# alibaba/pairec

Measured on AMD Instinct MI355X. Metric: ranked items/sec, 5k-cand DNN rank (recall top-5000 of 100M x 128 -> DNN3 -> fuse -> sort), higher is better.
Workload: dtype bf16x3; 1 GPU; configs[1]+[2]: recall 5k of 100000000x128 fp32 table in HBM -> 3-layer DNN rank (256-512-256-1, bf16 MFMA with split hi + lo operands = bf16x3, fp32-accurate scores) -> RankScore fusion (fp64) -> ItemRankScore sort; candidates_per_request=5000, table_rows=100000000, dim=128, table_dist=uniform, batches_in_flight=2, contexts=2, all_batches_on_predicted_thresholds=True, batches_re_run_after_a_failed_plan=0, parallelism=1 GPU

## Files before the change

pairec_amd/csrc/common.hpp:

```cpp
#pragma once
#include <hip/hip_runtime.h>

#include <algorithm>
#include <cstdarg>
#include <cstdint>
#include <cstdio>
#include <cstring>
#include <map>
#include <atomic>
#include <memory>
#include <mutex>
#include <shared_mutex>
#include <string>
#include <vector>

#include "../../include/pairec_gpu.h"

namespace pg {

struct PipeRun;
void set_error(const char* fmt, ...);

#define PG_HIP(expr)                                                                           \
    do {                                                                                       \
// ... 423 lines not shown
                      uint32_t* d_out_count);

int rank_dnn3_dev_locked(pg_ctx* ctx, const pg_model* m, const pg_table* t, const float* d_user,
                         const uint32_t* d_cand, const uint32_t* d_off, uint32_t n_req, uint32_t n_items,
                         float* d_out, size_t out_stride = 0);
int fm2t_user_embedding_locked(pg_ctx* ctx, const pg_model* m, const float* d_user, uint32_t n_req, float* d_out);
int rank_fm2t_irows_dev_locked(pg_ctx* ctx, const pg_model* m, const pg_item_rows* ir, const float* d_user, const int32_t* d_ufids,
                               const uint32_t* d_cand, const uint32_t* d_off, uint32_t n_req, uint32_t n_items, float* d_out);
int rank_fm2t_rows_dev_locked(pg_ctx* ctx, const pg_model* m, const pg_features* fs, const int32_t* item_field_cols,
                              const float* d_user, const int32_t* d_ufids, const uint32_t* d_cand, const uint32_t* d_off,
                              uint32_t n_req, uint32_t n_items, float* d_out);
int expr_eval_enqueue_locked(pg_ctx* ctx, const pg_expr* e, const double* d_vars, uint32_t n_items, double* d_out,
                             uint32_t* d_err, uint32_t items_per_flag);
void set_expr_arith_error(const pg_expr* e);
constexpr int kMaxRewrites = 8;
void expr_hold(const pg_expr* e);
void expr_release(const pg_expr* e);
struct ExprHold {
    const pg_expr* e = nullptr;
    ExprHold() = default;
    ExprHold(const ExprHold&) = delete;
    ExprHold& operator=(const ExprHold&) = delete;
    void take(const pg_expr* x) {
        if (e) expr_release(e);
        e = x;
        if (e) expr_hold(e);
    }
    ~ExprHold() { if (e) expr_release(e); }
};
int expr_num_rewrites(const pg_expr* e);
const char* expr_rewrite_source(const pg_expr* e, int r);
int expr_rewrite_num_vars(const pg_expr* e, int r);
const char* expr_rewrite_var_name(const pg_expr* e, int r, int i);
int expr_rewrite_eval_enqueue_locked(pg_ctx* ctx, const pg_expr* e, int r, const double* d_vars, uint32_t n_items, double* d_out,
                                     uint32_t* d_err, uint32_t items_per_flag);
int table_gather_locked(pg_ctx* ctx, const pg_table* t, const uint32_t* d_rows, uint32_t n, float* d_out);
int dpp_run_locked(pg_ctx* ctx, const float* d_emb32, const double* d_hook, const double* d_rel, uint32_t R, uint32_t n,
                   uint32_t d, uint32_t hook_dim, double alpha, uint32_t topn, uint32_t window, int normalize,
                   int ensure_pos, int has_table, uint32_t* d_out, uint32_t* d_out_count, double* d_L_out = nullptr);
int sort_dev_locked(pg_ctx* ctx, const double* d_scores, const uint32_t* d_seg, uint32_t n_seg, uint32_t n_items,
                    uint32_t max_seg, int desc, uint32_t* d_out);

void pipe_pool_destroy(pg_ctx* ctx);
int scratch_reserve(pg_ctx* ctx, int slot, size_t bytes, void** out);
template <class T>
int recall_check(const char* who, const pg_ctx* ctx, const T* over, const void* queries, const void* rows, const void* scores, uint32_t nq,
                 uint32_t k, bool l2) {
    PG_REQUIRE(ctx && over && queries && rows && scores, "%s: NULL argument", who);
    PG_REQUIRE(nq >= 1 && nq <= (uint32_t)kMaxQueries, "%s: nq=%u must be in [1,%d]", who, nq, kMaxQueries);
    PG_REQUIRE(l2 || over->dim <= 128 || nq <= 32, "%s: dim %u supports at most 32 queries per call", who, over->dim);
    if (k < 1 || k > 16384) {
        set_error("%s: k=%u unsupported (1..16384)", who, k);
        return PG_ERR_UNSUPPORTED;
    }
    return PG_OK;
}
template <class Run>
int recall_staged(pg_ctx* ctx, uint32_t dim, const float* queries, uint32_t nq, uint32_t k, uint64_t* out_rows, float* out_scores, Run&& run) {
    void* buf;
    int rc;
    const size_t qb = (size_t)nq * dim * 4, rb = (size_t)nq * k * 8, sb = (size_t)nq * k * 4;
    if ((rc = scratch_reserve(ctx, 5, qb + rb + sb + 64, &buf))) return rc;
    float* d_q = (float*)buf;
    uint64_t* d_rows = (uint64_t*)((char*)buf + ((qb + 15) & ~(size_t)15));
    float* d_sc = (float*)((char*)d_rows + rb);
    PG_HIP(hipMemcpyAsync(d_q, queries, qb, hipMemcpyHostToDevice, ctx->stream));
    if ((rc = run(d_q, d_rows, d_sc))) return rc;
    PG_HIP(hipMemcpyAsync(out_rows, d_rows, rb, hipMemcpyDeviceToHost, ctx->stream));
// ... 9 lines not shown
```

pairec_amd/csrc/expr.hip:

```cpp
#include "common.hpp"

#include <cmath>
#include <string>
#include <vector>

namespace pg {

enum OpCode : uint32_t { OP_CONST = 0, OP_VAR, OP_ADD, OP_SUB, OP_MUL, OP_DIV, OP_MOD, OP_POW, OP_FNZ,
                         OP_DIVF,
                         OP_NEG };

struct Instr {
    uint32_t op;
    uint32_t arg;
    double val;
};

constexpr int kMaxStack = 32;
constexpr int kMaxProg = 128;

}

struct pg_expr {
    std::string source;
// ... 233 lines not shown
    if (xfin && x != 0.0 && x != 1.0 && y != 0.0 && ay < 9223372036854775808.0 && ay == trunc(ay)) {
        double a1 = 1.0;
        long long ae = 0;
        int xe_i;
        double x1 = frexp(x, &xe_i);
        long long xe = xe_i;
        for (long long i = (long long)ay; i != 0; i >>= 1) {
            if (xe < -(1ll << 12) || (1ll << 12) < xe) {
                ae += xe;
                break;
            }
            if (i & 1) {
                a1 *= x1;
                ae += xe;
            }
            x1 *= x1;
            xe <<= 1;
            if (x1 < 0.5) {
                x1 += x1;
                xe--;
            }
        }
        if (y < 0.0) {
            a1 = 1.0 / a1;
            ae = -ae;
        }
        if (ae > 4096) ae = 4096;
        if (ae < -4096) ae = -4096;
        return ldexp(a1, (int)ae);
    }
    return pow(x, y);
}

__global__ void expr_eval_kernel(ExprDev e, const double* __restrict__ vars, uint32_t n_items,
                                 double* __restrict__ out, uint32_t* __restrict__ err, uint32_t items_per_flag) {
    const uint32_t i = blockIdx.x * blockDim.x + threadIdx.x;
    if (i >= n_items) return;
    double st[kMaxStack];
    int sp = 0;
    bool bad = false;
    for (uint32_t pc = 0; pc < e.n; ++pc) {
        const Instr in = e.prog[pc];
        if (in.op == OP_CONST) {
            st[sp++] = in.val;
        } else if (in.op == OP_VAR) {
            st[sp++] = vars[(size_t)in.arg * n_items + i];
        } else {
            if (in.op == OP_NEG) {
                st[sp - 1] = -st[sp - 1];
                continue;
            }
            const double r = st[--sp];
            const double l = st[--sp];
            double v = 0.0;
            switch (in.op) {
                case OP_DIVF: v = l / r; break;
                case OP_ADD: v = l + r; break;
                case OP_SUB: v = l - r; break;
                case OP_MUL: v = l * r; break;
                case OP_DIV:
                    if (r == 0.0) bad = true; else v = l / r;
                    break;
                case OP_MOD: {
                    const long long li = (l == l && fabs(l) < 9223372036854775808.0) ? (long long)l : (long long)0x8000000000000000ull;
                    const long long ri = (r == r && fabs(r) < 9223372036854775808.0) ? (long long)r : (long long)0x8000000000000000ull;
                    if (ri == 0) bad = true;
                    else if (ri == -1) v = 0.0;
                    else v = (double)(li % ri);
                    break;
                }
                case OP_POW: v = go_pow(l, r); break;
                case OP_FNZ: v = (l != 0.0) ? l : r; break;
            }
            st[sp++] = v;
        }
    }
    out[i] = sp > 0 ? st[sp - 1] : 0.0;
    if (bad) atomicOr(err + (items_per_flag ? i / items_per_flag : 0u), 1u);
}

int expr_eval_enqueue_locked(pg_ctx* ctx, const pg_expr* e, const double* d_vars, uint32_t n_items, double* d_out,
                             uint32_t* d_err, uint32_t items_per_flag) {
    if (e->empty) {
        PG_HIP(hipMemsetAsync(d_out, 0, (size_t)n_items * 8, ctx->stream));
    } else {
        ExprDev dev;
        dev.n = (uint32_t)e->prog.size();
        for (size_t i = 0; i < e->prog.size(); ++i) dev.prog[i] = e->prog[i];
        expr_eval_kernel<<<(n_items + 255) / 256, 256, 0, ctx->stream>>>(dev, d_vars, n_items, d_out, d_err, items_per_flag);
        PG_HIP(hipGetLastError());
    }
    return PG_OK;
}

int expr_num_rewrites(const pg_expr* e) { return e ? (int)e->rewrites.size() : 0; }
const char* expr_rewrite_source(const pg_expr* e, int r) { return e->rewrites[(size_t)r].source.c_str(); }
int expr_rewrite_num_vars(const pg_expr* e, int r) { return (int)e->rewrites[(size_t)r].vars.size(); }
const char* expr_rewrite_var_name(const pg_expr* e, int r, int i) { return e->rewrites[(size_t)r].vars[(size_t)i].c_str(); }
int expr_rewrite_eval_enqueue_locked(pg_ctx* ctx, const pg_expr* e, int r, const double* d_vars, uint32_t n_items, double* d_out,
                                     uint32_t* d_err, uint32_t items_per_flag) {
    const pg_expr::Rewrite& rw = e->rewrites[(size_t)r];
    if (rw.failed || rw.prog.empty()) {
        PG_HIP(hipMemsetAsync(d_out, 0, (size_t)n_items * 8, ctx->stream));
        return PG_OK;
    }
    ExprDev dev;
    dev.n = (uint32_t)rw.prog.size();
    for (size_t i = 0; i < rw.prog.size(); ++i) dev.prog[i] = rw.prog[i];
    expr_eval_kernel<<<(n_items + 255) / 256, 256, 0, ctx->stream>>>(dev, d_vars, n_items, d_out, d_err, items_per_flag);
    PG_HIP(hipGetLastError());
    return PG_OK;
}

void set_expr_arith_error(const pg_expr* e) {
    set_error("pg_expr_eval: violation of arithmetic specification: a division by zero in '%s' "
              "(the reference panics in ExprASTResult, utils/ast/ast.go:243-249)", e->source.c_str());
}

static int expr_eval_locked(pg_ctx* ctx, const pg_expr* e, const double* d_vars, uint32_t n_items,
                            double* d_out) {
    void* p;
    int rc;
    if ((rc = scratch_reserve(ctx, 4, 4096, &p))) return rc;
    uint32_t* d_err = (uint32_t*)p + 320;
    PG_HIP(hipMemsetAsync(d_err, 0, 4, ctx->stream));
    if ((rc = expr_eval_enqueue_locked(ctx, e, d_vars, n_items, d_out, d_err, 0))) return rc;
    PG_HIP(hipMemcpyAsync(ctx->h_status + 320, d_err, 4, hipMemcpyDeviceToHost, ctx->stream));
    PG_HIP(hipStreamSynchronize(ctx->stream));
    if (ctx->h_status[320] != 0) {
        set_expr_arith_error(e);
        return PG_ERR_ARITH;
    }
    return PG_OK;
}

struct ExprCol {
    const void* base;
    int32_t dtype;
    int32_t pad;
    double def;
};
struct ExprCols16 { ExprCol c[16]; };
// ... 353 lines not shown
```

pairec_amd/csrc/misc.hip:

```cpp
#include "pipeline.hpp"

#include <algorithm>
#include <cstring>
#include <vector>

namespace pg {

__global__ void rows_to_local_kernel(const uint64_t* __restrict__ rows, uint32_t n, uint64_t off,
                                     uint64_t nrows, uint32_t* __restrict__ local,
                                     uint8_t* __restrict__ owned, uint32_t* __restrict__ uni_off, uint32_t uni_nq, uint32_t uni_k) {
    const uint32_t i = blockIdx.x * blockDim.x + threadIdx.x;
    if (uni_off && i <= uni_nq) uni_off[i] = i * uni_k;
    if (i >= n) return;
    const uint64_t r = rows[i];
    const bool mine = r != ~0ull && r >= off && r - off < nrows;
    local[i] = mine ? (uint32_t)(r - off) : 0u;
    if (owned) owned[i] = mine ? 1 : 0;
}

__global__ void widen_kernel(const float* __restrict__ in, uint32_t n, double* __restrict__ out) {
    const uint32_t i = blockIdx.x * blockDim.x + threadIdx.x;
    if (i < n) out[i] = (double)in[i];
}

typedef uint32_t u32x4 __attribute__((ext_vector_type(4)));
__global__ __launch_bounds__(256) void hbm_probe_kernel(const u32x4* __restrict__ p, uint64_t n16,
                                                        uint32_t* __restrict__ sink) {
    uint32_t acc = 0;
    const uint64_t stride = (uint64_t)gridDim.x * blockDim.x;
    uint64_t i = (uint64_t)blockIdx.x * blockDim.x + threadIdx.x;
    for (; i + 3 * stride < n16; i += 4 * stride) {
        const u32x4 a = __builtin_nontemporal_load(&p[i]);
        const u32x4 b = __builtin_nontemporal_load(&p[i + stride]);
        const u32x4 c = __builtin_nontemporal_load(&p[i + 2 * stride]);
        const u32x4 d = __builtin_nontemporal_load(&p[i + 3 * stride]);
        acc ^= a.x ^ a.y ^ a.z ^ a.w ^ b.x ^ b.y ^ b.z ^ b.w ^ c.x ^ c.y ^ c.z ^ c.w ^ d.x ^ d.y ^ d.z ^ d.w;
    }
    for (; i < n16; i += stride) {
        const u32x4 a = __builtin_nontemporal_load(&p[i]);
        acc ^= a.x ^ a.y ^ a.z ^ a.w;
    }
    if (acc == 0x9E3779B9u) *sink = acc;
}

__global__ void uniform_offsets_kernel(uint32_t nq, uint32_t k, uint32_t* __restrict__ off) {
// ... 53 lines not shown
    sorted_head_kernel<<<(nq * C + 255) / 256, 256, 0, st>>>(d_order, d_rows, d_fused, nq, k, C, d_c_rows, d_c_rel);
    PG_HIP(hipGetLastError());
    return PG_OK;
}

int gather_global_rows_launch(hipStream_t st, const pg_table* t, const uint64_t* d_global_rows, uint32_t n, float* d_out) {
    if (n == 0) return PG_OK;
    const uint64_t threads = (uint64_t)n * (t->dim / 4);
    gather_global_rows_kernel<<<(uint32_t)((threads + 255) / 256), 256, 0, st>>>(t->d, t->dim, t->row_offset, t->rows, d_global_rows, n, d_out);
    PG_HIP(hipGetLastError());
    return PG_OK;
}

size_t page_entry_bytes(int n_algos) { return 20 + 4 * (size_t)n_algos; }

int page_launch(hipStream_t st, const uint32_t* d_order, const uint32_t* d_pick, const uint32_t* d_pick_cnt,
                const uint64_t* d_rows, const float* d_recall, const float* d_rank, size_t rank_stride, int n_algos,
                const double* d_fused, uint32_t nq, uint32_t k, uint32_t top_n, char* d_page) {
    const size_t np = (size_t)nq * top_n;
    if (np == 0) return PG_OK;
    uint64_t* p_rows = (uint64_t*)d_page;
    double* p_fused = (double*)(p_rows + np);
    float* p_recall = (float*)(p_fused + np);
    float* p_rank = p_recall + np;
    page_kernel<<<(uint32_t)((np + 255) / 256), 256, 0, st>>>(d_order, d_pick, d_pick_cnt, d_rows, d_recall, d_rank, rank_stride, n_algos,
                                                             d_fused, nq, k, top_n, p_rows, p_fused, p_recall, p_rank);
    PG_HIP(hipGetLastError());
    return PG_OK;
}

int rows_to_local_locked(pg_ctx* ctx, const pg_table* t, const uint64_t* d_rows, uint32_t n, uint32_t* d_local,
                         uint8_t* d_owned) {
    if (n == 0) return PG_OK;
    rows_to_local_kernel<<<(n + 255) / 256, 256, 0, ctx->stream>>>(d_rows, n, t->row_offset, t->rows, d_local, d_owned, nullptr, 0, 0);
    PG_HIP(hipGetLastError());
    return PG_OK;
}

int rows_to_local_offsets_locked(pg_ctx* ctx, const pg_table* t, const uint64_t* d_rows, uint32_t nq, uint32_t k, uint32_t* d_local,
                                 uint32_t* d_off) {
    const uint32_t n = nq * k;
    if (n <= nq) {
        int rc = uniform_offsets_locked(ctx, nq, k, d_off);
        return rc ? rc : rows_to_local_locked(ctx, t, d_rows, n, d_local, nullptr);
    }
    rows_to_local_kernel<<<(n + 255) / 256, 256, 0, ctx->stream>>>(d_rows, n, t->row_offset, t->rows, d_local, nullptr, d_off, nq, k);
    PG_HIP(hipGetLastError());
    return PG_OK;
}

int uniform_offsets_locked(pg_ctx* ctx, uint32_t nq, uint32_t k, uint32_t* d_off) {
    uniform_offsets_kernel<<<(nq + 256) / 256, 256, 0, ctx->stream>>>(nq, k, d_off);
    PG_HIP(hipGetLastError());
    return PG_OK;
}

}

extern "C" {

int pg_hbm_read_probe(pg_ctx* ctx, const pg_table* t, int reps, double* out_gbps) {
    PG_REQUIRE(ctx && t && out_gbps && reps > 0, "pg_hbm_read_probe: bad argument");
    const void* d_buf = t->d;
    const uint64_t bytes = t->rows * (uint64_t)t->dim * 4;
    PG_REQUIRE(bytes >= (1u << 20), "pg_hbm_read_probe: table smaller than 1 MiB");
    std::lock_guard<std::mutex> g(ctx->mu);
    void* sink;
    int rc;
    if ((rc = pg::scratch_reserve(ctx, 4, 4096, &sink))) return rc;
    const uint64_t n16 = bytes / 16;
    const int grid = ctx->num_cus * 8;
    double best = 0.0;
    for (int r = 0; r < reps + 1; ++r) {
        PG_HIP(hipEventRecord(ctx->ev[0], ctx->stream));
        pg::hbm_probe_kernel<<<grid, 256, 0, ctx->stream>>>((const pg::u32x4*)d_buf, n16, (uint32_t*)sink + 900);
        PG_HIP(hipGetLastError());
        PG_HIP(hipEventRecord(ctx->ev[1], ctx->stream));
        PG_HIP(hipStreamSynchronize(ctx->stream));
        float ms = 0.f;
// ... 27 lines not shown
```

pairec_amd/csrc/pipeline.hip:

```cpp
#include "pipeline.hpp"

#include <algorithm>
#include <chrono>
#include <thread>

namespace pg {

struct VarSrc { int8_t src[32]; };
__global__ void bind_vars_kernel(const float* __restrict__ recall, const float* __restrict__ rank, size_t rank_stride,
                                 uint32_t n, uint32_t nv, VarSrc vs, double* __restrict__ vars, uint32_t* __restrict__ err,
                                 const double* __restrict__ rw, int zero_err) {
    const uint32_t i = blockIdx.x * blockDim.x + threadIdx.x;
    if (zero_err && i < (uint32_t)kMaxQueries) err[i] = 0;
    if (i >= n) return;
    const double a = (double)recall[i];
    for (uint32_t v = 0; v < nv; ++v) {
        const int sa = vs.src[v];
        vars[(size_t)v * n + i] = sa >= 0 ? (double)rank[(size_t)sa * rank_stride + i] : (sa == -1 ? a : rw[(size_t)(-2 - sa) * n + i]);
    }
}

__global__ void mask_pads_kernel(const uint64_t* __restrict__ rows, uint32_t n, float* __restrict__ rank, size_t rank_stride,
                                 int n_algos, double* __restrict__ fused) {
    const uint32_t i = blockIdx.x * blockDim.x + threadIdx.x;
    if (i >= n || rows[i] != ~0ull) return;
    for (int a = 0; a < n_algos; ++a) rank[(size_t)a * rank_stride + i] = 0.0f;
    fused[i] = __longlong_as_double(0x7FF8000000000000ll);
}

int pipe_run_acquire(pg_ctx* ctx, PipeRun** out) {
    {
        std::lock_guard<std::mutex> g(ctx->pool_mu);
        if (!ctx->pipe_free.empty()) {
            *out = ctx->pipe_free.back();
            ctx->pipe_free.pop_back();
            return PG_OK;
        }
    }
    PG_HIP(hipSetDevice(ctx->device));
    PipeRun* r = new PipeRun();
    if (hipHostMalloc((void**)&r->h_status, kPipeStatusWords * 4) != hipSuccess || hipEventCreate(&r->done) != hipSuccess) {
        set_error("pipeline: cannot allocate a batch's status block: %s", hipGetErrorString(hipGetLastError()));
        if (r->h_status) hipHostFree(r->h_status);
        delete r;
        return PG_ERR_DEVICE;
    }
    *out = r;
    return PG_OK;
}

void pipe_run_release(pg_ctx* ctx, PipeRun* r) {
    std::lock_guard<std::mutex> g(ctx->pool_mu);
    ctx->pipe_free.push_back(r);
// ... 31 lines not shown
        int found = -2;
        bool rewritten = false;
        for (int r = 0; r < n_rw; ++r)
            if (!strcmp(name, expr_rewrite_source(e, r))) {
                found = -2 - r;
                rewritten = true;
            }
        if (!rewritten && (found = plane_of(name)) == -2) {
            set_error("%s: RankScore variable \"%s\" is neither a rank algorithm of the scene, a ScoreRewrite source nor current_score", who, name);
            return PG_ERR_INVALID;
        }
        var_src->push_back(found);
    }
    for (int r = 0; r < n_rw; ++r)
        for (int i = 0; i < expr_rewrite_num_vars(e, r); ++i) {
            const char* name = expr_rewrite_var_name(e, r, i);
            const int found = plane_of(name);
            if (found == -2) {
                set_error("%s: ScoreRewrite[\"%s\"] variable \"%s\" is neither a rank algorithm of the scene nor current_score", who,
                          expr_rewrite_source(e, r), name);
                return PG_ERR_INVALID;
            }
            var_src->push_back(found);
        }
    return PG_OK;
}

int post_scratch(pg_ctx* ctx, const RecommendCall& c, uint32_t nq, PostScratch* ps) {
    const uint32_t n = nq * c.k;
    void* buf;
    int rc;
    auto al = [](size_t x) { return (x + 255) & ~(size_t)255; };
    const size_t b_local = al((size_t)n * 4), b_off = al((size_t)(nq + 1) * 4), b_err = al((size_t)kMaxQueries * 4);
    int wide = std::max(c.nv, 1);
    const int n_rw = expr_num_rewrites(c.e);
    for (int r = 0; r < n_rw; ++r) wide = std::max(wide, expr_rewrite_num_vars(c.e, r));
    const size_t b_vars = al((size_t)(wide + n_rw) * n * 8);
    if ((rc = scratch_reserve(ctx, 8, b_local + b_off + b_err + b_vars, &buf))) return rc;
    ps->d_local = (uint32_t*)buf;
    ps->d_off = (uint32_t*)((char*)buf + b_local);
    ps->d_err = (uint32_t*)((char*)buf + b_local + b_off);
    ps->d_vars = (double*)((char*)buf + b_local + b_off + b_err);
    ps->c_rows = nullptr; ps->c_rel = nullptr; ps->c_emb = nullptr; ps->c_bail = nullptr;
    if (c.rerank.kind) {
        const size_t nc = (size_t)nq * c.rerank.candidates;
        const size_t b_rows = al(nc * 8), b_rel = al(nc * 8), b_emb = al(nc * c.t->dim * 4), b_bail = al((size_t)kMaxQueries * 4);
        if ((rc = scratch_reserve(ctx, 10, b_rows + b_rel + b_emb + b_bail, &buf))) return rc;
        ps->c_rows = (uint64_t*)buf;
        ps->c_rel = (double*)((char*)buf + b_rows);
        ps->c_emb = (float*)((char*)buf + b_rows + b_rel);
        ps->c_bail = (uint32_t*)((char*)buf + b_rows + b_rel + b_emb);
    }
    return PG_OK;
}

int fuse_scores_enqueue_locked(pg_ctx* ctx, const pg_expr* e, const int* var_src, int nv, const float* d_recall, const float* d_rank,
                               size_t rank_stride, uint32_t n, uint32_t items_per_flag, double* d_vars, uint32_t* d_err, double* d_fused) {
    hipStream_t st = ctx->stream;
    int rc;
    VarSrc vs;
    const int n_rw = expr_num_rewrites(e);
    int wide = std::max(nv, 1);
    for (int r = 0; r < n_rw; ++r) wide = std::max(wide, expr_rewrite_num_vars(e, r));
    double* const d_rw = d_vars + (size_t)wide * n;
    const uint32_t bind_grid = (std::max(n, (uint32_t)kMaxQueries) + 255) / 256;
    bool zeroed = false;
    for (int r = 0, at = nv; r < n_rw; ++r) {
        const int nvr = expr_rewrite_num_vars(e, r);
        for (int i = 0; i < 32; ++i) vs.src[i] = i < nvr ? (int8_t)var_src[at + i] : (int8_t)-1;
        at += nvr;
        if (nvr > 0 || !zeroed) {
            bind_vars_kernel<<<bind_grid, 256, 0, st>>>(d_recall, d_rank, rank_stride, n, (uint32_t)nvr, vs, d_vars, d_err, nullptr, zeroed ? 0 : 1);
            PG_HIP(hipGetLastError());
            zeroed = true;
        }
        if ((rc = expr_rewrite_eval_enqueue_locked(ctx, e, r, d_vars, n, d_rw + (size_t)r * n, d_err, items_per_flag))) return rc;
    }
    for (int i = 0; i < 32; ++i) vs.src[i] = i < nv ? (int8_t)var_src[i] : (int8_t)-1;
    if (nv > 0) {
        bind_vars_kernel<<<bind_grid, 256, 0, st>>>(d_recall, d_rank, rank_stride, n, (uint32_t)nv, vs, d_vars, d_err, d_rw, zeroed ? 0 : 1);
        PG_HIP(hipGetLastError());
    } else if (!zeroed) {
        PG_HIP(hipMemsetAsync(d_err, 0, (size_t)kMaxQueries * 4, st));
    }
    return expr_eval_enqueue_locked(ctx, e, d_vars, n, d_fused, d_err, items_per_flag);
}

int post_fuse_sort_locked(pg_ctx* ctx, const RecommendCall& c, uint32_t q0, uint32_t nq, const PostScratch& ps) {
    const uint32_t n = nq * c.k;
    const size_t o = (size_t)q0 * c.k;
    hipStream_t st = ctx->stream;
    int rc;
    if ((rc = fuse_scores_enqueue_locked(ctx, c.e, c.var_src, c.nv, c.d_recall + o, c.d_rank + o, c.rank_stride, n, c.k, ps.d_vars, ps.d_err,
                                         c.d_fused + o)))
        return rc;
    if (c.pads) {
        mask_pads_kernel<<<(n + 255) / 256, 256, 0, st>>>(c.d_rows + o, n, c.d_rank + o, c.rank_stride, c.planes(), c.d_fused + o);
        PG_HIP(hipGetLastError());
    }
    return sort_dev_locked(ctx, c.d_fused + o, ps.d_off, nq, n, c.k, 1, c.d_order + o);
}

int rerank_select_locked(pg_ctx* ctx, const RecommendCall& c, uint32_t q0, uint32_t nq, const PostScratch& ps) {
    const uint32_t C = c.rerank.candidates;
    const size_t o = (size_t)q0 * c.k;
    if (c.k < C) {
        set_error("recommend: the DPP stage wants %u candidates, the lists hold k = %u", C, c.k);
        return PG_ERR_UNSUPPORTED;
    }
    int rc;
    if ((rc = sorted_head_launch(ctx->stream, c.d_order + o, c.d_rows + o, c.d_fused + o, nq, c.k, C, ps.c_rows, ps.c_rel))) return rc;
    return dpp_norm_relevance_launch(ctx->stream, ps.c_rel, nq, C, c.rerank.dpp.norm_relevance_score, ps.c_bail);
}
int rerank_run_locked(pg_ctx* ctx, const RecommendCall& c, uint32_t q0, uint32_t nq, const PostScratch& ps) {
    const uint32_t C = c.rerank.candidates;
    int rc;
    if ((rc = dpp_run_locked(ctx, ps.c_emb, nullptr, ps.c_rel, nq, C, c.t->dim, 0, c.rerank.dpp.alpha, c.top_n, c.rerank.dpp.window,
                             c.rerank.dpp.normalize_emb, 1, 1, c.d_pick + (size_t)q0 * c.top_n, c.d_pick_cnt + q0)))
        return rc;
    if (c.rerank.dpp.norm_relevance_score)
        return dpp_bail_fix_launch(ctx->stream, ps.c_bail, nq, C, c.top_n, c.d_pick + (size_t)q0 * c.top_n, c.d_pick_cnt + q0);
    return PG_OK;
}

static int recommend_post_locked(pg_ctx* ctx, const RecommendCall& c, uint32_t q0, uint32_t nq, const PostScratch& ps) {
    const uint32_t n = nq * c.k;
    const size_t o = (size_t)q0 * c.k;
    int rc;
    if ((rc = rows_to_local_offsets_locked(ctx, c.t, c.d_rows + o, nq, c.k, ps.d_local, ps.d_off))) return rc;
    for (int a = 0; a < c.n_algos; ++a) {
        const RankAlgoRef& al = c.algos[a];
        float* out = c.d_rank + (size_t)c.plane0[a] * c.rank_stride + o;
        const float* users = c.d_queries + (size_t)q0 * c.t->dim;
        if ((rc = rank_algo_locked(ctx, al, c.t, users, c.d_ufids ? c.d_ufids + (size_t)q0 * c.ufid_stride : nullptr, ps.d_local, ps.d_off, nq, n,
                                   out, c.rank_stride)))
            return rc;
    }
    if ((rc = post_fuse_sort_locked(ctx, c, q0, nq, ps))) return rc;
    if (c.rerank.kind == 1) {
        if (c.t->rows < c.rerank.candidates) {
            set_error("recommend: the DPP stage wants %u candidates, the table has %llu rows", c.rerank.candidates, (unsigned long long)c.t->rows);
            return PG_ERR_UNSUPPORTED;
        }
        if ((rc = rerank_select_locked(ctx, c, q0, nq, ps))) return rc;
        if ((rc = gather_global_rows_launch(ctx->stream, c.t, ps.c_rows, nq * c.rerank.candidates, ps.c_emb))) return rc;
        if ((rc = rerank_run_locked(ctx, c, q0, nq, ps))) return rc;
    }
    return PG_OK;
}

int rank_algo_locked(pg_ctx* ctx, const RankAlgoRef& al, const pg_table* t, const float* d_user, const int32_t* d_ufids,
                     const uint32_t* d_cand, const uint32_t* d_off, uint32_t n_req, uint32_t n_items, float* d_out, size_t out_stride) {
    if (al.m->kind == PG_MODEL_DNN3) return rank_dnn3_dev_locked(ctx, al.m, t, d_user, d_cand, d_off, n_req, n_items, d_out, out_stride);
    if (al.irows) return rank_fm2t_irows_dev_locked(ctx, al.m, al.irows, d_user, d_ufids, d_cand, d_off, n_req, n_items, d_out);
    return rank_fm2t_rows_dev_locked(ctx, al.m, al.fs, al.item_field_cols, d_user, d_ufids, d_cand, d_off, n_req, n_items, d_out);
}

int recommend_enqueue(pg_ctx* ctx, const RecommendCall& c, PipeRun* r, bool first) {
    if (c.t->d_row_map) {
        set_error("recommend: the table is a filtered view (pg_table_view_create) — views serve the recall calls only");
        return PG_ERR_UNSUPPORTED;
    }
    std::lock_guard<std::mutex> g(ctx->mu);
    TimersScope quiet(ctx, c.timers);
    TableRead tr(c.t->rw);
    int rc;
    PostScratch ps;
    if ((rc = post_scratch(ctx, c, c.nq, &ps))) return rc;
    r->patched = false;
    if (!first && r->job.table_gen != c.t->generation.load(std::memory_order_relaxed)) first = true;
    if (first) {
// ... 99 lines not shown
        if (hipEventSynchronize(tk->run->done) != hipSuccess) {
            pg::set_error("pg_recommend_end: %s", hipGetErrorString(hipGetLastError()));
            rc = PG_ERR_DEVICE;
            break;
        }
        if ((rc = pg::recommend_verify(ctx, tk->run, &ok, &tk->call))) break;
        if (!ok && (rc = pg::recommend_enqueue(ctx, tk->call, tk->run, false))) break;
    }
    if (!rc) {
        if (scan_ms) *scan_ms = tk->run->job.scan_ms;
        for (uint32_t q = 0; q < tk->call.nq; ++q)
            if (tk->run->h_status[pg::kExprFlagAt + q]) {
                pg::set_expr_arith_error(tk->call.e);
                rc = PG_ERR_ARITH;
                break;
            }
    }
    pg::pipe_run_release(ctx, tk->run);
    delete tk;
    return rc;
}

int pg_fuse_scores_dev(pg_ctx* ctx, const pg_expr* e, const char* const* plane_names, uint32_t n_planes, const float* d_rank,
                       size_t rank_stride, const float* d_recall, uint32_t n, double* d_fused) {
    PG_REQUIRE(ctx && e && (n_planes == 0 || (plane_names && d_rank)) && d_recall && d_fused, "pg_fuse_scores_dev: NULL argument");
    PG_REQUIRE(n_planes <= (uint32_t)pg::kMaxPlanes, "pg_fuse_scores_dev: %u planes (at most %d)", n_planes, pg::kMaxPlanes);
    if (n == 0) return PG_OK;
    std::vector<int> var_src;
    pg::ExprHold hold;
    hold.take(e);
    int rc;
    if ((rc = pg::recommend_bind_vars(e, plane_names, (int)n_planes, &var_src, "pg_fuse_scores_dev"))) return rc;
    const int nv = pg_expr_num_vars(e), n_rw = pg::expr_num_rewrites(e);
    int wide = std::max(nv, 1);
    for (int r = 0; r < n_rw; ++r) wide = std::max(wide, pg::expr_rewrite_num_vars(e, r));
    std::lock_guard<std::mutex> g(ctx->mu);
    void* buf;
    const size_t b_vars = (((size_t)(wide + n_rw) * n * 8) + 255) & ~(size_t)255;
    if ((rc = pg::scratch_reserve(ctx, 15, b_vars + (size_t)pg::kMaxQueries * 4, &buf))) return rc;
    double* const d_vars = (double*)buf;
    uint32_t* const d_err = (uint32_t*)((char*)buf + b_vars);
    if ((rc = pg::fuse_scores_enqueue_locked(ctx, e, var_src.data(), nv, d_recall, d_rank, rank_stride, n, 0u, d_vars, d_err, d_fused))) return rc;
    PG_HIP(hipMemcpyAsync(ctx->h_status + 321, d_err, 4, hipMemcpyDeviceToHost, ctx->stream));
    PG_HIP(hipStreamSynchronize(ctx->stream));
    if (ctx->h_status[321] != 0) {
        pg::set_expr_arith_error(e);
        return PG_ERR_ARITH;
    }
    return PG_OK;
}

int pg_recommend_end_timed(pg_ctx* ctx, pg_ticket* tk, uint32_t timeout_us, double* scan_ms) {
    PG_REQUIRE(ctx && tk, "pg_recommend_end_timed: NULL argument");
    if (timeout_us) {
        const auto deadline = std::chrono::steady_clock::now() + std::chrono::microseconds(timeout_us);
        for (;;) {
            const hipError_t q = hipEventQuery(tk->run->done);
            if (q == hipSuccess) break;
            if (q != hipErrorNotReady) {
                pg::set_error("pg_recommend_end_timed: %s", hipGetErrorString(q));
                return PG_ERR_DEVICE;
            }
            if (std::chrono::steady_clock::now() >= deadline) {
                pg::set_error("pg_recommend_end_timed: the batch did not complete within %u us (the ticket stays valid)", timeout_us);
                return PG_ERR_TIMEOUT;
            }
            std::this_thread::sleep_for(std::chrono::microseconds(50));
        }
    }
    return pg_recommend_end(ctx, tk, scan_ms);
}

int pg_recommend_dnn3_dev(pg_ctx* ctx, const pg_table* t, const pg_model* m, const pg_expr* e, const char* rank_var,
                          const float* d_queries, uint32_t nq, uint32_t k, uint64_t* d_out_rows,
                          float* d_out_recall_scores, float* d_out_rank_scores, double* d_out_fused,
// ... 11 lines not shown
```

pairec_amd/csrc/pipeline.hpp:

```cpp
#pragma once
#include "common.hpp"

namespace pg {

struct RecommendCall;
struct PipeRun {
    RecallJob job;
    uint32_t* h_status = nullptr;
    std::vector<hipEvent_t> events;
    hipEvent_t done = nullptr;
    bool patched = false;
};
constexpr uint32_t kExprFlagAt = 320;
constexpr uint32_t kPipeStatusWords = 640;

int pipe_run_acquire(pg_ctx* ctx, PipeRun** out);
void pipe_run_release(pg_ctx* ctx, PipeRun* r);

constexpr int kMaxAlgos = 4;
struct RankAlgoRef {
    const pg_model* m = nullptr;
    const pg_features* fs = nullptr;
    int32_t item_field_cols[16] = {0};
    const pg_item_rows* irows = nullptr;
// ... 11 lines not shown
struct RecommendCall {
    bool timers = true;
    const pg_table* t = nullptr;
    RankAlgoRef algos[kMaxAlgos];
    int n_algos = 0;
    const pg_expr* e = nullptr;
    const int* var_src = nullptr;
    int nv = 0;
    const float* d_queries = nullptr;
    const int32_t* d_ufids = nullptr;
    uint32_t ufid_stride = 0;
    uint32_t nq = 0, k = 0;
    uint64_t* d_rows = nullptr;
    float* d_recall = nullptr;
    float* d_rank = nullptr;
    size_t rank_stride = 0;
    int plane0[kMaxAlgos] = {0, 1, 2, 3};
    int n_planes = 0;
    int planes() const { return n_planes ? n_planes : n_algos; }
    double* d_fused = nullptr;
    uint32_t* d_order = nullptr;
    uint32_t* d_count = nullptr;
    bool pads = false;
    RerankStage rerank;
    uint32_t top_n = 0;
    uint32_t* d_pick = nullptr;
    uint32_t* d_pick_cnt = nullptr;
};
int recommend_bind_vars(const pg_expr* e, const char* const* names, int n_algos, std::vector<int>* var_src, const char* who);
int recommend_enqueue(pg_ctx* ctx, const RecommendCall& c, PipeRun* r, bool first);
int recommend_verify(pg_ctx* ctx, PipeRun* r, bool* ok, const RecommendCall* c = nullptr);
struct PostScratch {
    uint32_t *d_local, *d_off, *d_err;
    double* d_vars;
    uint64_t* c_rows;
    double* c_rel;
    float* c_emb;
    uint32_t* c_bail;
};
int post_scratch(pg_ctx* ctx, const RecommendCall& c, uint32_t nq, PostScratch* ps);
int post_fuse_sort_locked(pg_ctx* ctx, const RecommendCall& c, uint32_t q0, uint32_t nq, const PostScratch& ps);
int fuse_scores_enqueue_locked(pg_ctx* ctx, const pg_expr* e, const int* var_src, int nv, const float* d_recall, const float* d_rank,
                               size_t rank_stride, uint32_t n, uint32_t items_per_flag, double* d_vars, uint32_t* d_err, double* d_fused);
int rerank_select_locked(pg_ctx* ctx, const RecommendCall& c, uint32_t q0, uint32_t nq, const PostScratch& ps);
int rerank_run_locked(pg_ctx* ctx, const RecommendCall& c, uint32_t q0, uint32_t nq, const PostScratch& ps);

int rows_to_local_locked(pg_ctx* ctx, const pg_table* t, const uint64_t* d_rows, uint32_t n, uint32_t* d_local,
                         uint8_t* d_owned);
int uniform_offsets_locked(pg_ctx* ctx, uint32_t nq, uint32_t k, uint32_t* d_off);
int rows_to_local_offsets_locked(pg_ctx* ctx, const pg_table* t, const uint64_t* d_rows, uint32_t nq, uint32_t k, uint32_t* d_local,
                                 uint32_t* d_off);
int sorted_head_launch(hipStream_t st, const uint32_t* d_order, const uint64_t* d_rows, const double* d_fused, uint32_t nq,
                       uint32_t k, uint32_t C, uint64_t* d_c_rows, double* d_c_rel);
int gather_global_rows_launch(hipStream_t st, const pg_table* t, const uint64_t* d_global_rows, uint32_t n, float* d_out);
size_t page_entry_bytes(int n_algos);
int page_launch(hipStream_t st, const uint32_t* d_order, const uint32_t* d_pick, const uint32_t* d_pick_cnt,
                const uint64_t* d_rows, const float* d_recall, const float* d_rank, size_t rank_stride, int n_algos,
                const double* d_fused, uint32_t nq, uint32_t k, uint32_t top_n, char* d_page);
int dpp_norm_relevance_launch(hipStream_t st, double* d_rel, uint32_t nq, uint32_t n, int mode, uint32_t* d_bail);
int dpp_bail_fix_launch(hipStream_t st, const uint32_t* d_bail, uint32_t nq, uint32_t n, uint32_t top_n, uint32_t* d_pick,
                        uint32_t* d_pick_cnt);
bool dpp_norm_relevance_host(const double* rel, uint32_t n, int mode, double* out);
int ssd_run_locked(pg_ctx* ctx, const pg_table* t, const uint32_t* d_cand, const double* d_rel, uint32_t R, uint32_t n,
                   double gamma, uint32_t T, uint32_t window, int normalize_emb, int ensure_pos_similarity, int use_ssd_star,
                   uint32_t* d_out);
bool ssd_batchable(uint32_t d1, uint32_t window);
bool ssd_norm_quality_host(const double* rel, uint32_t n, int mode, double* out);

}
```

Measured before the change: 271.0 million ranked items/s.

## Fuse variable binding into expression eval kernel and fold error zeroing into rows_to_local

Removes the separate bind_vars kernel that materialized every expression variable as an fp64 array. The expression evaluator now loads each variable directly from the recall/rank float planes or the rewrite outputs through a source map. Zeroing of the error flags is folded into the rows_to_local kernel, so it no longer needs its own memset or kernel. This saves kernel launches and the HBM write and read-back of the variable arrays. The catch is a per-variable branch and indirect load inside the interpreter loop.

```diff
diff --git a/pairec_amd/csrc/common.hpp b/pairec_amd/csrc/common.hpp
--- a/pairec_amd/csrc/common.hpp
+++ b/pairec_amd/csrc/common.hpp
@@ -479,8 +479,15 @@
 const char* expr_rewrite_source(const pg_expr* e, int r);
 int expr_rewrite_num_vars(const pg_expr* e, int r);
 const char* expr_rewrite_var_name(const pg_expr* e, int r, int i);
-int expr_rewrite_eval_enqueue_locked(pg_ctx* ctx, const pg_expr* e, int r, const double* d_vars, uint32_t n_items, double* d_out,
-                                     uint32_t* d_err, uint32_t items_per_flag);
+struct ExprBind {
+    const float* recall;
+    const float* rank;
+    size_t rank_stride;
+    const double* rw;
+    int8_t src[32];
+};
+int expr_eval_bound_enqueue_locked(pg_ctx* ctx, const pg_expr* e, int r, const ExprBind& b, uint32_t n_items, double* d_out,
+                                   uint32_t* d_err, uint32_t items_per_flag);
 int table_gather_locked(pg_ctx* ctx, const pg_table* t, const uint32_t* d_rows, uint32_t n, float* d_out);
 int dpp_run_locked(pg_ctx* ctx, const float* d_emb32, const double* d_hook, const double* d_rel, uint32_t R, uint32_t n,
                    uint32_t d, uint32_t hook_dim, double alpha, uint32_t topn, uint32_t window, int normalize,
diff --git a/pairec_amd/csrc/expr.hip b/pairec_amd/csrc/expr.hip
--- a/pairec_amd/csrc/expr.hip
+++ b/pairec_amd/csrc/expr.hip
@@ -289,10 +289,9 @@
     return pow(x, y);
 }
 
-__global__ void expr_eval_kernel(ExprDev e, const double* __restrict__ vars, uint32_t n_items,
-                                 double* __restrict__ out, uint32_t* __restrict__ err, uint32_t items_per_flag) {
-    const uint32_t i = blockIdx.x * blockDim.x + threadIdx.x;
-    if (i >= n_items) return;
+template <class Load>
+__device__ __forceinline__ void expr_eval_item(const ExprDev& e, uint32_t i, Load load, double* __restrict__ out,
+                                               uint32_t* __restrict__ err, uint32_t items_per_flag) {
     double st[kMaxStack];
     int sp = 0;
     bool bad = false;
@@ -301,7 +300,7 @@
         if (in.op == OP_CONST) {
             st[sp++] = in.val;
         } else if (in.op == OP_VAR) {
-            st[sp++] = vars[(size_t)in.arg * n_items + i];
+            st[sp++] = load(in.arg);
         } else {
             if (in.op == OP_NEG) {
                 st[sp - 1] = -st[sp - 1];
@@ -336,6 +335,23 @@
     if (bad) atomicOr(err + (items_per_flag ? i / items_per_flag : 0u), 1u);
 }
 
+__global__ void expr_eval_kernel(ExprDev e, const double* __restrict__ vars, uint32_t n_items,
+                                 double* __restrict__ out, uint32_t* __restrict__ err, uint32_t items_per_flag) {
+    const uint32_t i = blockIdx.x * blockDim.x + threadIdx.x;
+    if (i >= n_items) return;
+    expr_eval_item(e, i, [&](uint32_t v) { return vars[(size_t)v * n_items + i]; }, out, err, items_per_flag);
+}
+
+__global__ void expr_eval_bound_kernel(ExprDev e, ExprBind b, uint32_t n_items, double* __restrict__ out,
+                                       uint32_t* __restrict__ err, uint32_t items_per_flag) {
+    const uint32_t i = blockIdx.x * blockDim.x + threadIdx.x;
+    if (i >= n_items) return;
+    expr_eval_item(e, i, [&](uint32_t v) {
+        const int sa = b.src[v & 31];
+        return sa >= 0 ? (double)b.rank[(size_t)sa * b.rank_stride + i] : (sa == -1 ? (double)b.recall[i] : b.rw[(size_t)(-2 - sa) * n_items + i]);
+    }, out, err, items_per_flag);
+}
+
 int expr_eval_enqueue_locked(pg_ctx* ctx, const pg_expr* e, const double* d_vars, uint32_t n_items, double* d_out,
                              uint32_t* d_err, uint32_t items_per_flag) {
     if (e->empty) {
@@ -354,17 +370,17 @@
 const char* expr_rewrite_source(const pg_expr* e, int r) { return e->rewrites[(size_t)r].source.c_str(); }
 int expr_rewrite_num_vars(const pg_expr* e, int r) { return (int)e->rewrites[(size_t)r].vars.size(); }
 const char* expr_rewrite_var_name(const pg_expr* e, int r, int i) { return e->rewrites[(size_t)r].vars[(size_t)i].c_str(); }
-int expr_rewrite_eval_enqueue_locked(pg_ctx* ctx, const pg_expr* e, int r, const double* d_vars, uint32_t n_items, double* d_out,
-                                     uint32_t* d_err, uint32_t items_per_flag) {
-    const pg_expr::Rewrite& rw = e->rewrites[(size_t)r];
-    if (rw.failed || rw.prog.empty()) {
+int expr_eval_bound_enqueue_locked(pg_ctx* ctx, const pg_expr* e, int r, const ExprBind& b, uint32_t n_items, double* d_out,
+                                   uint32_t* d_err, uint32_t items_per_flag) {
+    const std::vector<Instr>& prog = r < 0 ? e->prog : e->rewrites[(size_t)r].prog;
+    if (r < 0 ? e->empty : (e->rewrites[(size_t)r].failed || prog.empty())) {
         PG_HIP(hipMemsetAsync(d_out, 0, (size_t)n_items * 8, ctx->stream));
         return PG_OK;
     }
     ExprDev dev;
-    dev.n = (uint32_t)rw.prog.size();
-    for (size_t i = 0; i < rw.prog.size(); ++i) dev.prog[i] = rw.prog[i];
-    expr_eval_kernel<<<(n_items + 255) / 256, 256, 0, ctx->stream>>>(dev, d_vars, n_items, d_out, d_err, items_per_flag);
+    dev.n = (uint32_t)prog.size();
+    for (size_t i = 0; i < prog.size(); ++i) dev.prog[i] = prog[i];
+    expr_eval_bound_kernel<<<(n_items + 255) / 256, 256, 0, ctx->stream>>>(dev, b, n_items, d_out, d_err, items_per_flag);
     PG_HIP(hipGetLastError());
     return PG_OK;
 }
diff --git a/pairec_amd/csrc/misc.hip b/pairec_amd/csrc/misc.hip
--- a/pairec_amd/csrc/misc.hip
+++ b/pairec_amd/csrc/misc.hip
@@ -8,9 +8,11 @@
 
 __global__ void rows_to_local_kernel(const uint64_t* __restrict__ rows, uint32_t n, uint64_t off,
                                      uint64_t nrows, uint32_t* __restrict__ local,
-                                     uint8_t* __restrict__ owned, uint32_t* __restrict__ uni_off, uint32_t uni_nq, uint32_t uni_k) {
+                                     uint8_t* __restrict__ owned, uint32_t* __restrict__ uni_off, uint32_t uni_nq, uint32_t uni_k,
+                                     uint32_t* __restrict__ zero) {
     const uint32_t i = blockIdx.x * blockDim.x + threadIdx.x;
     if (uni_off && i <= uni_nq) uni_off[i] = i * uni_k;
+    if (zero && i < (uint32_t)kMaxQueries) zero[i] = 0;
     if (i >= n) return;
     const uint64_t r = rows[i];
     const bool mine = r != ~0ull && r >= off && r - off < nrows;
@@ -130,19 +132,20 @@
 int rows_to_local_locked(pg_ctx* ctx, const pg_table* t, const uint64_t* d_rows, uint32_t n, uint32_t* d_local,
                          uint8_t* d_owned) {
     if (n == 0) return PG_OK;
-    rows_to_local_kernel<<<(n + 255) / 256, 256, 0, ctx->stream>>>(d_rows, n, t->row_offset, t->rows, d_local, d_owned, nullptr, 0, 0);
+    rows_to_local_kernel<<<(n + 255) / 256, 256, 0, ctx->stream>>>(d_rows, n, t->row_offset, t->rows, d_local, d_owned, nullptr, 0, 0, nullptr);
     PG_HIP(hipGetLastError());
     return PG_OK;
 }
 
 int rows_to_local_offsets_locked(pg_ctx* ctx, const pg_table* t, const uint64_t* d_rows, uint32_t nq, uint32_t k, uint32_t* d_local,
-                                 uint32_t* d_off) {
+                                 uint32_t* d_off, uint32_t* d_zero) {
     const uint32_t n = nq * k;
     if (n <= nq) {
+        if (d_zero) PG_HIP(hipMemsetAsync(d_zero, 0, (size_t)kMaxQueries * 4, ctx->stream));
         int rc = uniform_offsets_locked(ctx, nq, k, d_off);
         return rc ? rc : rows_to_local_locked(ctx, t, d_rows, n, d_local, nullptr);
     }
-    rows_to_local_kernel<<<(n + 255) / 256, 256, 0, ctx->stream>>>(d_rows, n, t->row_offset, t->rows, d_local, nullptr, d_off, nq, k);
+    rows_to_local_kernel<<<(n + 255) / 256, 256, 0, ctx->stream>>>(d_rows, n, t->row_offset, t->rows, d_local, nullptr, d_off, nq, k, d_zero);
     PG_HIP(hipGetLastError());
     return PG_OK;
 }
diff --git a/pairec_amd/csrc/pipeline.hip b/pairec_amd/csrc/pipeline.hip
--- a/pairec_amd/csrc/pipeline.hip
+++ b/pairec_amd/csrc/pipeline.hip
@@ -5,20 +5,6 @@
 #include <thread>
 
 namespace pg {
-
-struct VarSrc { int8_t src[32]; };
-__global__ void bind_vars_kernel(const float* __restrict__ recall, const float* __restrict__ rank, size_t rank_stride,
-                                 uint32_t n, uint32_t nv, VarSrc vs, double* __restrict__ vars, uint32_t* __restrict__ err,
-                                 const double* __restrict__ rw, int zero_err) {
-    const uint32_t i = blockIdx.x * blockDim.x + threadIdx.x;
-    if (zero_err && i < (uint32_t)kMaxQueries) err[i] = 0;
-    if (i >= n) return;
-    const double a = (double)recall[i];
-    for (uint32_t v = 0; v < nv; ++v) {
-        const int sa = vs.src[v];
-        vars[(size_t)v * n + i] = sa >= 0 ? (double)rank[(size_t)sa * rank_stride + i] : (sa == -1 ? a : rw[(size_t)(-2 - sa) * n + i]);
-    }
-}
 
 __global__ void mask_pads_kernel(const uint64_t* __restrict__ rows, uint32_t n, float* __restrict__ rank, size_t rank_stride,
                                  int n_algos, double* __restrict__ fused) {
@@ -116,15 +102,12 @@
     int rc;
     auto al = [](size_t x) { return (x + 255) & ~(size_t)255; };
     const size_t b_local = al((size_t)n * 4), b_off = al((size_t)(nq + 1) * 4), b_err = al((size_t)kMaxQueries * 4);
-    int wide = std::max(c.nv, 1);
-    const int n_rw = expr_num_rewrites(c.e);
-    for (int r = 0; r < n_rw; ++r) wide = std::max(wide, expr_rewrite_num_vars(c.e, r));
-    const size_t b_vars = al((size_t)(wide + n_rw) * n * 8);
-    if ((rc = scratch_reserve(ctx, 8, b_local + b_off + b_err + b_vars, &buf))) return rc;
+    const size_t b_rw = al((size_t)expr_num_rewrites(c.e) * n * 8);
+    if ((rc = scratch_reserve(ctx, 8, b_local + b_off + b_err + b_rw, &buf))) return rc;
     ps->d_local = (uint32_t*)buf;
     ps->d_off = (uint32_t*)((char*)buf + b_local);
     ps->d_err = (uint32_t*)((char*)buf + b_local + b_off);
-    ps->d_vars = (double*)((char*)buf + b_local + b_off + b_err);
+    ps->d_rw = (double*)((char*)buf + b_local + b_off + b_err);
     ps->c_rows = nullptr; ps->c_rel = nullptr; ps->c_emb = nullptr; ps->c_bail = nullptr;
     if (c.rerank.kind) {
         const size_t nc = (size_t)nq * c.rerank.candidates;
@@ -139,44 +122,34 @@
 }
 
 int fuse_scores_enqueue_locked(pg_ctx* ctx, const pg_expr* e, const int* var_src, int nv, const float* d_recall, const float* d_rank,
-                               size_t rank_stride, uint32_t n, uint32_t items_per_flag, double* d_vars, uint32_t* d_err, double* d_fused) {
-    hipStream_t st = ctx->stream;
-    int rc;
-    VarSrc vs;
+                               size_t rank_stride, uint32_t n, uint32_t items_per_flag, double* d_rw, uint32_t* d_err, double* d_fused,
+                               bool err_zeroed) {
+    int rc;
+    ExprBind b;
+    b.recall = d_recall;
+    b.rank = d_rank;
+    b.rank_stride = rank_stride;
+    b.rw = nullptr;
+    if (!err_zeroed) PG_HIP(hipMemsetAsync(d_err, 0, (size_t)kMaxQueries * 4, ctx->stream));
     const int n_rw = expr_num_rewrites(e);
-    int wide = std::max(nv, 1);
-    for (int r = 0; r < n_rw; ++r) wide = std::max(wide, expr_rewrite_num_vars(e, r));
-    double* const d_rw = d_vars + (size_t)wide * n;
-    const uint32_t bind_grid = (std::max(n, (uint32_t)kMaxQueries) + 255) / 256;
-    bool zeroed = false;
     for (int r = 0, at = nv; r < n_rw; ++r) {
         const int nvr = expr_rewrite_num_vars(e, r);
-        for (int i = 0; i < 32; ++i) vs.src[i] = i < nvr ? (int8_t)var_src[at + i] : (int8_t)-1;
+        for (int i = 0; i < 32; ++i) b.src[i] = i < nvr ? (int8_t)var_src[at + i] : (int8_t)-1;
         at += nvr;
-        if (nvr > 0 || !zeroed) {
-            bind_vars_kernel<<<bind_grid, 256, 0, st>>>(d_recall, d_rank, rank_stride, n, (uint32_t)nvr, vs, d_vars, d_err, nullptr, zeroed ? 0 : 1);
-            PG_HIP(hipGetLastError());
-            zeroed = true;
-        }
-        if ((rc = expr_rewrite_eval_enqueue_locked(ctx, e, r, d_vars, n, d_rw + (size_t)r * n, d_err, items_per_flag))) return rc;
-    }
-    for (int i = 0; i < 32; ++i) vs.src[i] = i < nv ? (int8_t)var_src[i] : (int8_t)-1;
-    if (nv > 0) {
-        bind_vars_kernel<<<bind_grid, 256, 0, st>>>(d_recall, d_rank, rank_stride, n, (uint32_t)nv, vs, d_vars, d_err, d_rw, zeroed ? 0 : 1);
-        PG_HIP(hipGetLastError());
-    } else if (!zeroed) {
-        PG_HIP(hipMemsetAsync(d_err, 0, (size_t)kMaxQueries * 4, st));
-    }
-    return expr_eval_enqueue_locked(ctx, e, d_vars, n, d_fused, d_err, items_per_flag);
-}
-
-int post_fuse_sort_locked(pg_ctx* ctx, const RecommendCall& c, uint32_t q0, uint32_t nq, const PostScratch& ps) {
+        if ((rc = expr_eval_bound_enqueue_locked(ctx, e, r, b, n, d_rw + (size_t)r * n, d_err, items_per_flag))) return rc;
+    }
+    for (int i = 0; i < 32; ++i) b.src[i] = i < nv ? (int8_t)var_src[i] : (int8_t)-1;
+    b.rw = d_rw;
+    return expr_eval_bound_enqueue_locked(ctx, e, -1, b, n, d_fused, d_err, items_per_flag);
+}
+
+int post_fuse_sort_locked(pg_ctx* ctx, const RecommendCall& c, uint32_t q0, uint32_t nq, const PostScratch& ps, bool err_zeroed) {
     const uint32_t n = nq * c.k;
     const size_t o = (size_t)q0 * c.k;
     hipStream_t st = ctx->stream;
     int rc;
-    if ((rc = fuse_scores_enqueue_locked(ctx, c.e, c.var_src, c.nv, c.d_recall + o, c.d_rank + o, c.rank_stride, n, c.k, ps.d_vars, ps.d_err,
-                                         c.d_fused + o)))
+    if ((rc = fuse_scores_enqueue_locked(ctx, c.e, c.var_src, c.nv, c.d_recall + o, c.d_rank + o, c.rank_stride, n, c.k, ps.d_rw, ps.d_err,
+                                         c.d_fused + o, err_zeroed)))
         return rc;
     if (c.pads) {
         mask_pads_kernel<<<(n + 255) / 256, 256, 0, st>>>(c.d_rows + o, n, c.d_rank + o, c.rank_stride, c.planes(), c.d_fused + o);
@@ -211,7 +184,7 @@
     const uint32_t n = nq * c.k;
     const size_t o = (size_t)q0 * c.k;
     int rc;
-    if ((rc = rows_to_local_offsets_locked(ctx, c.t, c.d_rows + o, nq, c.k, ps.d_local, ps.d_off))) return rc;
+    if ((rc = rows_to_local_offsets_locked(ctx, c.t, c.d_rows + o, nq, c.k, ps.d_local, ps.d_off, ps.d_err))) return rc;
     for (int a = 0; a < c.n_algos; ++a) {
         const RankAlgoRef& al = c.algos[a];
         float* out = c.d_rank + (size_t)c.plane0[a] * c.rank_stride + o;
@@ -220,7 +193,7 @@
                                    out, c.rank_stride)))
             return rc;
     }
-    if ((rc = post_fuse_sort_locked(ctx, c, q0, nq, ps))) return rc;
+    if ((rc = post_fuse_sort_locked(ctx, c, q0, nq, ps, true))) return rc;
     if (c.rerank.kind == 1) {
         if (c.t->rows < c.rerank.candidates) {
             set_error("recommend: the DPP stage wants %u candidates, the table has %llu rows", c.rerank.candidates, (unsigned long long)c.t->rows);
@@ -386,15 +359,13 @@
     int rc;
     if ((rc = pg::recommend_bind_vars(e, plane_names, (int)n_planes, &var_src, "pg_fuse_scores_dev"))) return rc;
     const int nv = pg_expr_num_vars(e), n_rw = pg::expr_num_rewrites(e);
-    int wide = std::max(nv, 1);
-    for (int r = 0; r < n_rw; ++r) wide = std::max(wide, pg::expr_rewrite_num_vars(e, r));
     std::lock_guard<std::mutex> g(ctx->mu);
     void* buf;
-    const size_t b_vars = (((size_t)(wide + n_rw) * n * 8) + 255) & ~(size_t)255;
-    if ((rc = pg::scratch_reserve(ctx, 15, b_vars + (size_t)pg::kMaxQueries * 4, &buf))) return rc;
-    double* const d_vars = (double*)buf;
-    uint32_t* const d_err = (uint32_t*)((char*)buf + b_vars);
-    if ((rc = pg::fuse_scores_enqueue_locked(ctx, e, var_src.data(), nv, d_recall, d_rank, rank_stride, n, 0u, d_vars, d_err, d_fused))) return rc;
+    const size_t b_rw = (((size_t)n_rw * n * 8) + 255) & ~(size_t)255;
+    if ((rc = pg::scratch_reserve(ctx, 15, b_rw + (size_t)pg::kMaxQueries * 4, &buf))) return rc;
+    double* const d_rw = (double*)buf;
+    uint32_t* const d_err = (uint32_t*)((char*)buf + b_rw);
+    if ((rc = pg::fuse_scores_enqueue_locked(ctx, e, var_src.data(), nv, d_recall, d_rank, rank_stride, n, 0u, d_rw, d_err, d_fused, false))) return rc;
     PG_HIP(hipMemcpyAsync(ctx->h_status + 321, d_err, 4, hipMemcpyDeviceToHost, ctx->stream));
     PG_HIP(hipStreamSynchronize(ctx->stream));
     if (ctx->h_status[321] != 0) {
diff --git a/pairec_amd/csrc/pipeline.hpp b/pairec_amd/csrc/pipeline.hpp
--- a/pairec_amd/csrc/pipeline.hpp
+++ b/pairec_amd/csrc/pipeline.hpp
@@ -67,16 +67,17 @@
 int recommend_verify(pg_ctx* ctx, PipeRun* r, bool* ok, const RecommendCall* c = nullptr);
 struct PostScratch {
     uint32_t *d_local, *d_off, *d_err;
-    double* d_vars;
+    double* d_rw;
     uint64_t* c_rows;
     double* c_rel;
     float* c_emb;
     uint32_t* c_bail;
 };
 int post_scratch(pg_ctx* ctx, const RecommendCall& c, uint32_t nq, PostScratch* ps);
-int post_fuse_sort_locked(pg_ctx* ctx, const RecommendCall& c, uint32_t q0, uint32_t nq, const PostScratch& ps);
+int post_fuse_sort_locked(pg_ctx* ctx, const RecommendCall& c, uint32_t q0, uint32_t nq, const PostScratch& ps, bool err_zeroed = false);
 int fuse_scores_enqueue_locked(pg_ctx* ctx, const pg_expr* e, const int* var_src, int nv, const float* d_recall, const float* d_rank,
-                               size_t rank_stride, uint32_t n, uint32_t items_per_flag, double* d_vars, uint32_t* d_err, double* d_fused);
+                               size_t rank_stride, uint32_t n, uint32_t items_per_flag, double* d_rw, uint32_t* d_err, double* d_fused,
+                               bool err_zeroed);
 int rerank_select_locked(pg_ctx* ctx, const RecommendCall& c, uint32_t q0, uint32_t nq, const PostScratch& ps);
 int rerank_run_locked(pg_ctx* ctx, const RecommendCall& c, uint32_t q0, uint32_t nq, const PostScratch& ps);
 
@@ -84,7 +85,7 @@
                          uint8_t* d_owned);
 int uniform_offsets_locked(pg_ctx* ctx, uint32_t nq, uint32_t k, uint32_t* d_off);
 int rows_to_local_offsets_locked(pg_ctx* ctx, const pg_table* t, const uint64_t* d_rows, uint32_t nq, uint32_t k, uint32_t* d_local,
-                                 uint32_t* d_off);
+                                 uint32_t* d_off, uint32_t* d_zero = nullptr);
 int sorted_head_launch(hipStream_t st, const uint32_t* d_order, const uint64_t* d_rows, const double* d_fused, uint32_t nq,
                        uint32_t k, uint32_t C, uint64_t* d_c_rows, double* d_c_rel);
 int gather_global_rows_launch(hipStream_t st, const pg_table* t, const uint64_t* d_global_rows, uint32_t n, float* d_out);
```

Measured after the change: 270.8 million ranked items/s, median of 2. Within noise of the previous version (-0.0%).
